# dselivanov/rsparse

Hardware: AMD Instinct MI355X
Metric: als_iterations_per_sec (higher is better)
Workload: dtype f32 (Gram products of rows > 512 / <= 32 non-zeros as 2 x fp16 / 3 x bf16 split terms of the fp32 operands, fp32 accumulate; everything else fp32)

## Files before the change

### rsparse_amd/csrc/wrmf_cgq.hip

```cpp
#include <algorithm>
#include <cstdlib>

#include "wrmf_internal.h"
#include "wrmf_device.h"

namespace rsparse_hip {
namespace {

using namespace dev;

typedef float f32x2 __attribute__((ext_vector_type(2)));

#ifndef RSP_ZPAD_MINCAPQ
#define RSP_ZPAD_MINCAPQ 0
#endif
#ifndef RSP_TSAVE_MINCAPQ
#define RSP_TSAVE_MINCAPQ 0
#endif
#ifndef RSP_GVFIRST_MINCAPQ
#define RSP_GVFIRST_MINCAPQ 16
#endif
#ifndef RSP_STREAM_IDX_PREFETCH
#define RSP_STREAM_IDX_PREFETCH 1
#endif
#ifndef RSP_IDX_PREFETCH_MAXWPR
#define RSP_IDX_PREFETCH_MAXWPR 2
#endif
#ifndef RSP_STREAM_PREFIX_Q
#define RSP_STREAM_PREFIX_Q 4
#endif

constexpr float kCgTolQ = 1e-10f;
constexpr int kMaxSavedSweeps = 4;

template <int KP>
struct QG {
  static constexpr int RPN = KP / 16;
  static constexpr int VW = RPN >= 4 ? 4 : RPN;
  static constexpr int NV = RPN / VW;
  __device__ static __forceinline__ int elem(int i, int r) { return (r / VW) * (16 * VW) + i * VW + (r % VW); }
};

template <int VW>
struct Piece;
template <>
struct Piece<4> { using type = float4; };
template <>
struct Piece<2> { using type = float2; };

__device__ __forceinline__ float row16_sum(float v) {
  v += dpp<0xB1>(v);
  v += dpp<0x4E>(v);
  v += dpp<0x141>(v);
  v += dpp<0x140>(v);
  return v;
}
__device__ __forceinline__ float groups_sum(float v) {
  {
    const unsigned u = __float_as_uint(v);
    const auto r = __builtin_amdgcn_permlane16_swap(u, u, false, false);
    v = __uint_as_float(r[0]) + __uint_as_float(r[1]);
  }
  {
    const unsigned u = __float_as_uint(v);
    const auto r = __builtin_amdgcn_permlane32_swap(u, u, false, false);
    v = __uint_as_float(r[0]) + __uint_as_float(r[1]);
  }
  return v;
}

__device__ __forceinline__ float groups_reduce_scatter4(const float a0, const float a1, const float a2, const float a3) {
  const auto s01 = __builtin_amdgcn_permlane16_swap(__float_as_uint(a0), __float_as_uint(a1), false, false);
  const float c = __uint_as_float(s01[0]) + __uint_as_float(s01[1]);
  const auto s23 = __builtin_amdgcn_permlane16_swap(__float_as_uint(a2), __float_as_uint(a3), false, false);
  const float d = __uint_as_float(s23[0]) + __uint_as_float(s23[1]);
  const auto t = __builtin_amdgcn_permlane32_swap(__float_as_uint(c), __float_as_uint(d), false, false);
  return __uint_as_float(t[0]) + __uint_as_float(t[1]);
}
__device__ __forceinline__ void groups_all_gather4(const float r, float& o0, float& o1, float& o2, float& o3) {
  const unsigned u = __float_as_uint(r);
  const auto h = __builtin_amdgcn_permlane32_swap(u, u, false, false);
  const auto lo = __builtin_amdgcn_permlane16_swap(h[0], h[0], false, false);
  const auto hi = __builtin_amdgcn_permlane16_swap(h[1], h[1], false, false);
  o0 = __uint_as_float(lo[0]);
  o1 = __uint_as_float(lo[1]);
  o2 = __uint_as_float(hi[0]);
  o3 = __uint_as_float(hi[1]);
}
#ifndef RSP_NO_GRS
#define RSP_GRS 1
#else
#define RSP_GRS 0
#endif

typedef _Float16 f16x2 __attribute__((ext_vector_type(2)));
typedef _Float16 f16x8 __attribute__((ext_vector_type(8)));
typedef float f32x4 __attribute__((ext_vector_type(4)));
__device__ __forceinline__ int fp16_scale_exp(float vmax) {
  const int eb = (int)((__float_as_uint(vmax) >> 23) & 0xffu);
  return min(253, max(1, 267 - eb));
}
__device__ __forceinline__ void split_f16(const float x0, const float x1, unsigned& hi, unsigned& lo) {
  const f32x2 v = {x0, x1};
  const f16x2 h = __builtin_convertvector(v, f16x2);
  const f32x2 r = v - __builtin_convertvector(h, f32x2);
  const f16x2 l = __builtin_convertvector(r, f16x2);
  hi = __builtin_bit_cast(unsigned, h);
  lo = __builtin_bit_cast(unsigned, l);
}
__device__ __forceinline__ float row16_max(float v) {
  v = fmaxf(v, dpp<0xB1>(v));
  v = fmaxf(v, dpp<0x4E>(v));
  v = fmaxf(v, dpp<0x141>(v));
  v = fmaxf(v, dpp<0x140>(v));
  return v;
}

__device__ __forceinline__ unsigned lds_addr(const void* p) {
  return (unsigned)(reinterpret_cast<uintptr_t>(p));
}
__device__ __forceinline__ void dma4(const void* g, unsigned lds_base) {
  asm volatile("s_mov_b32 m0, %1\n\ts_nop 0\n\tglobal_load_lds_dword %0, off" : : "v"(g), "s"(lds_base) : "memory", "m0");
}
__device__ __forceinline__ void wait_vm0() { asm volatile("s_waitcnt vmcnt(0)" ::: "memory"); }

template <int KP, int CAPQ, int WAVES, int WPR, int STREAM, bool IMPLICIT, int DMF = 0>
struct QSmem {
  static constexpr size_t gram_floats = (IMPLICIT && DMF != 1) ? (size_t)KP * KP : 0;
  static constexpr size_t vec_floats = IMPLICIT ? (size_t)WAVES * KP : 0;
  static constexpr size_t red_floats = WPR > 1 ? (size_t)2 * WAVES * KP + 2 * WAVES : 0;
  static constexpr size_t tsv_floats = (STREAM && !(RSP_STREAM_IDX_PREFETCH && IMPLICIT)) ? 0 : (size_t)WAVES * 2 * CAPQ * 4;
  static constexpr size_t pre_floats = STREAM ? (size_t)WAVES * RSP_STREAM_PREFIX_Q * 4 * KP : 0;
  static constexpr int dmf_ps = KP + 8, dmf_os = KP + 4;
  static constexpr size_t dmf_floats = DMF ? (size_t)WAVES * dmf_ps + (size_t)WAVES * dmf_os : 0;
  static constexpr size_t pfx_floats = (!STREAM && WPR > RSP_IDX_PREFETCH_MAXWPR && CAPQ * 4 == 64) ? (size_t)WAVES * 2 * 64 : 0;
  static constexpr size_t bytes = (gram_floats + vec_floats + red_floats + tsv_floats + pre_floats + dmf_floats + pfx_floats) * 4 + 16;
};

template <int KP, int CAPQ, int WAVES, int WPR, int STREAM, bool IMPLICIT, int DMF = 0, bool GB = false, bool KFULL = false>
__global__ __launch_bounds__(WAVES * 64, 2) void als_cgq_kernel(AlsArgs a, const int32_t* __restrict__ rows, int n_rows,
                                                             int rows_per_team, size_t loss_slot0) {
  using G_ = QG<KP>;
  constexpr int RPN = G_::RPN, VW = G_::VW, NV = G_::NV, CAP = CAPQ * 4, TEAMS = WAVES / WPR;
  using piece_t = typename Piece<VW>::type;
  using SM = QSmem<KP, CAPQ, WAVES, WPR, STREAM, IMPLICIT, DMF>;
  static_assert(WAVES % WPR == 0, "teams must tile the workgroup");
  constexpr bool GRS = RSP_GRS && RPN == 8 && VW == 4;
  auto groups_all_reduce8 = [](float(&a8)[RPN]) {
    if constexpr (RPN == 8) {
      const float r0 = groups_reduce_scatter4(a8[0], a8[1], a8[2], a8[3]);
      const float r1 = groups_reduce_scatter4(a8[4], a8[5], a8[6], a8[7]);
      groups_all_gather4(r0, a8[0], a8[1], a8[2], a8[3]);
      groups_all_gather4(r1, a8[4], a8[5], a8[6], a8[7]);
    }
  };
  static_assert(!DMF || (IMPLICIT && KP == 128 && WAVES == 4 && WPR == 1 && STREAM == 0), "DMF geometry");
  static_assert(DMF != 1 || CAPQ == 8, "register-resident G terms: only the 8-quad kernel has the 64 registers");
  static_assert(!GB || IMPLICIT, "the global bias of explicit feedback is removed from the data (R/model_WRMF.R:278-282)");
  const float gbias = GB ? a.gbias : 0.f, ltgt = GB ? a.loss_tgt_const : 1.f;
  extern __shared__ __attribute__((aligned(16))) char smem[];
  float* sG = reinterpret_cast<float*>(smem);
  float* sVec = sG + SM::gram_floats;
  float* sRed = sVec + SM::vec_floats;
  float* sRedL = sRed + (WPR > 1 ? 2 * WAVES * KP : 0);
  float* sTsv = sVec + SM::vec_floats + SM::red_floats;
  float* sPre = sTsv + SM::tsv_floats;
  float* sPfx = sPre + SM::pre_floats;
  _Float16* sPh = reinterpret_cast<_Float16*>(sPre + SM::pre_floats);
  _Float16* sPl = sPh + WAVES * SM::dmf_ps;
  float* sOut = reinterpret_cast<float*>(sPl + WAVES * SM::dmf_ps);

  const int tid = threadIdx.x, lane = tid & 63, wv = rfl(tid >> 6);
  const int g = lane >> 4, i = lane & 15;
  const int team = wv / WPR, tw = wv % WPR;
  const int k = KFULL ? KP : a.k;
  if constexpr (IMPLICIT && DMF == 0) {
    constexpr int GU = (KP * KP) % (8 * WAVES * 64) == 0 ? 8 : ((KP * KP) % (2 * WAVES * 64) == 0 ? 2 : 1);
    static_assert((KP * KP) % (GU * WAVES * 64) == 0, "the Gramian copy walks whole batches");
    for (int e0 = tid; e0 < KP * KP; e0 += GU * WAVES * 64) {
      float gv[GU];
#pragma unroll
      for (int u = 0; u < GU; u++) {
        const int e = e0 + u * WAVES * 64, r = e / KP, c = e % KP;
        gv[u] = a.XtX[(size_t)min(r, k - 1) * k + min(c, k - 1)];
      }
#pragma unroll
      for (int u = 0; u < GU; u++) {
        const int e = e0 + u * WAVES * 64, r = e / KP, c = e % KP;
        sG[e] = (r < k && c < k) ? gv[u] : 0.f;
      }
    }
  }
  for (int e = tid; e < (int)(SM::vec_floats + SM::red_floats + SM::tsv_floats); e += WAVES * 64) sVec[e] = 0.f;
  __syncthreads();

  constexpr int NRES = (IMPLICIT && CAPQ == 8 && WPR == 1 && !STREAM && KP == 128 && !DMF) ? 2 : 0;
  piece_t gres[NRES > 0 ? NRES : 1][4][NV];
  if constexpr (NRES > 0) {
#pragma unroll
    for (int rs = 0; rs < NRES; rs++)
#pragma unroll
      for (int u = 0; u < 4; u++)
#pragma unroll
        for (int b = 0; b < NV; b++)
          gres[rs][u][b] = *reinterpret_cast<const piece_t*>(sG + (4 * (g + 4 * rs) + u) * KP + b * 16 * VW + i * VW);
  }
  f16x8 gAh[DMF == 1 ? 2 : 1][DMF == 1 ? 4 : 1], gAl[DMF == 1 ? 2 : 1][DMF == 1 ? 4 : 1];
  char* sGf = reinterpret_cast<char*>(sG) + (size_t)wv * 16 * 1024;
  float ginv = 1.f;
  if constexpr (DMF) {
    const int m = lane & 15, kb = lane >> 4;
    float gmax = 0.f;
#pragma unroll
    for (int t = 0; t < 2; t++)
#pragma unroll
      for (int ks = 0; ks < 4; ks++)
#pragma unroll
        for (int e = 0; e < 8; e++) {
          const int r = 32 * wv + 16 * t + m, c = 32 * ks + 8 * kb + e;
          {
            const float gv = a.XtX[(size_t)min(r, k - 1) * k + min(c, k - 1)];
            gmax = fmaxf(gmax, fabsf(gv) * ((r < k && c < k) ? 1.f : 0.f));
          }
        }
    for (int o = 32; o > 0; o >>= 1) gmax = fmaxf(gmax, __shfl_xor(gmax, o));
    const int ge = fp16_scale_exp(gmax);
    const float gs = __uint_as_float((unsigned)ge << 23);
    ginv = __uint_as_float((unsigned)(254 - ge) << 23);
#pragma unroll
    for (int t = 0; t < 2; t++)
#pragma unroll
      for (int ks = 0; ks < 4; ks++) {
        unsigned hi[4], lo[4];
#pragma unroll
        for (int e = 0; e < 8; e += 2) {
          const int r = 32 * wv + 16 * t + m, c = 32 * ks + 8 * kb + e;
          const float g0v = a.XtX[(size_t)min(r, k - 1) * k + min(c, k - 1)];
          const float g0 = g0v * ((r < k && c < k) ? 1.f : 0.f);
          const float g1v = a.XtX[(size_t)min(r, k - 1) * k + min(c + 1, k - 1)];
          const float g1 = g1v * ((r < k && c + 1 < k) ? 1.f : 0.f);
          split_f16(g0 * gs, g1 * gs, hi[e / 2], lo[e / 2]);
        }
        const uint4 h4 = {hi[0], hi[1], hi[2], hi[3]}, l4 = {lo[0], lo[1], lo[2], lo[3]};
        if constexpr (DMF == 1) {
          gAh[t][ks] = __builtin_bit_cast(f16x8, h4);
          gAl[t][ks] = __builtin_bit_cast(f16x8, l4);
        } else {
          *reinterpret_cast<uint4*>(sGf + ((t * 4 + ks) * 2 + 0) * 1024 + lane * 16) = h4;
          *reinterpret_cast<uint4*>(sGf + ((t * 4 + ks) * 2 + 1) * 1024 + lane * 16) = l4;
        }
      }
    if constexpr (DMF == 2) wave_sync();
  }
  float* vec = sVec + wv * KP;
  float* tacc = sTsv + wv * 2 * CAP;
  float* tcur = tacc + CAP;
  int buf = 0;
  double wloss = 0.0;
#ifdef RSP_CGQ_PROF
  unsigned long long cq_t[6] = {0, 0, 0, 0, 0, 0};
  unsigned long long cq_l = __builtin_amdgcn_s_memtime();
#define CQ_T(j) { const unsigned long long t1_ = __builtin_amdgcn_s_memtime(); cq_t[j] += t1_ - cq_l; cq_l = t1_; }
#else
#define CQ_T(j)
#endif
  int pf_id = 0, pf_cnt = -1;
  float pf_c = 0.f;
  const int team_global = blockIdx.x * TEAMS + team;
  const int total_teams = gridDim.x * TEAMS;

  auto row_index = [&](int itn) { return team_global + itn * total_teams; };
  int row_c = 0, p1_c = 0, p2_c = 0, row_n = 0;
  if (rows_per_team > 0 && row_index(0) < n_rows) {
    row_c = rows[row_index(0)];
    p1_c = a.col_ptrs[row_c];
    p2_c = a.col_ptrs[row_c + 1];
  }
  if (rows_per_team > 1 && row_index(1) < n_rows) row_n = rows[row_index(1)];
  for (int it = 0; it < rows_per_team; ++it) {
    const int ri = row_index(it);
    const bool have = ri < n_rows;
    if (WPR == 1 && !DMF && !have) break;
    const int row = have ? rfl(row_c) : 0;
    const int p1 = have ? rfl(p1_c) : 0;
    const int p2 = have ? rfl(p2_c) : 0;
    {
      int p1_n = 0, p2_n = 0, row_nn = 0;
      if (it + 1 < rows_per_team && row_index(it + 1) < n_rows) {
        p1_n = a.col_ptrs[row_n];
        p2_n = a.col_ptrs[row_n + 1];
      }
      if (it + 2 < rows_per_team && row_index(it + 2) < n_rows) row_nn = rows[row_index(it + 2)];
      row_c = row_n;
      p1_c = p1_n;
      p2_c = p2_n;
      row_n = row_nn;
    }
    const int cnt = p2 - p1;
    float* yrow = a.Y + (size_t)row * k;
    if (!GB && WPR == 1 && cnt <= 0) {
      if (!DMF || have)
        for (int e = lane; e < k; e += 64) yrow[e] = 0.f;
      if constexpr (!DMF) continue;
    }
    constexpr int PQ = STREAM ? RSP_STREAM_PREFIX_Q : 0, PCAP = PQ * 4, PTEAM = PCAP * WPR;
    const int pre = STREAM ? min(cnt, PTEAM) : 0;
    const int pw = STREAM ? max(0, min(PCAP, pre - tw * PCAP)) : 0;
    const int nchunks = (cnt - pre + CAP - 1) / CAP;
    constexpr bool resident = STREAM == 0;
    const float lam_use =
        IMPLICIT ? 0.f : (float)(a.lambda_loss * (a.dynamic_lambda ? (double)(float)cnt : 1.0));

    float* tscr = nullptr;
    float alph[kMaxSavedSweeps];
#pragma unroll
    for (int s2 = 0; s2 < kMaxSavedSweeps; s2++) alph[s2] = 0.f;
    if constexpr (STREAM == 1) {
      if (a.tscr && have && a.cg_steps <= kMaxSavedSweeps) tscr = a.tscr + a.stream_off[ri];
    }

    float xt[CAPQ][RPN];
    float cv[CAPQ];
    constexpr int NSL = (CAP + 63) / 64;
    float cl[NSL];
#pragma unroll
    for (int s2 = 0; s2 < NSL; s2++) cl[s2] = 0.f;
    int ccnt = 0;

    constexpr bool ZPAD = STREAM == 0 && CAPQ >= RSP_ZPAD_MINCAPQ;
    constexpr bool TSAVE = STREAM == 0 && CAPQ >= RSP_TSAVE_MINCAPQ;
    constexpr bool GVFIRST = STREAM == 0 && CAPQ >= RSP_GVFIRST_MINCAPQ;
    constexpr bool IDXPF = CAP <= 64 && ((STREAM == 0 && WPR <= RSP_IDX_PREFETCH_MAXWPR) || (STREAM == 1 && IMPLICIT && RSP_STREAM_IDX_PREFETCH));
#ifdef RSP_NO_DMAPF
    constexpr bool DMAPF = false;
#else
    constexpr bool DMAPF = KFULL && !IDXPF && SM::pfx_floats > 0;
#endif
    int* pfxI = reinterpret_cast<int*>(sPfx) + wv * 128;
    float* pfxC = sPfx + wv * 128 + 64;
    int pf_pos = -1;
    auto gather_q = [&](auto nq_tag, const int base, const int n, const bool from_pf = false) {
      constexpr int NQG = decltype(nq_tag)::value;
      int id[NQG > 0 ? NQG : 1];
      if constexpr (DMAPF) {
        if (!from_pf && n > 0) {
          const int j = base + min(lane, n - 1);
          dma4(a.row_idx + j, lds_addr(pfxI));
          dma4(a.vals + j, lds_addr(pfxC));
          wait_vm0();
        }
        wave_sync();
#pragma unroll
        for (int q = 0; q < NQG; q++) {
          const int j = max(min(4 * q + g, n - 1), 0);
          id[q] = pfxI[j];
          cv[q] = (!ZPAD || 4 * q + g < n) ? pfxC[j] : 0.f;
        }
        if constexpr (TSAVE) cl[0] = lane < n ? pfxC[lane] : 0.f;
        wave_sync();
      } else if (IDXPF && from_pf) {
        int* xi = reinterpret_cast<int*>(tacc);
        wave_sync();
        xi[lane & (CAP - 1)] = pf_id;
        tcur[lane & (CAP - 1)] = pf_c;
        wave_sync();
#pragma unroll
        for (int q = 0; q < NQG; q++) {
          const int j = max(min(4 * q + g, n - 1), 0);
          id[q] = xi[j];
          cv[q] = (!ZPAD || 4 * q + g < n) ? tcur[j] : 0.f;
        }
        if constexpr (TSAVE) cl[0] = lane < n ? pf_c : 0.f;
        wave_sync();
      } else {
#pragma unroll
        for (int q = 0; q < NQG; q++) {
          const int j = max(min(4 * q + g, n - 1), 0);
          id[q] = a.row_idx[base + j];
          const float c = a.vals[base + j];
          cv[q] = (!ZPAD || 4 * q + g < n) ? c : 0.f;
        }
        if constexpr (TSAVE) {
#pragma unroll
          for (int s2 = 0; s2 < NSL; s2++) cl[s2] = lane + 64 * s2 < n ? a.vals[base + lane + 64 * s2] : 0.f;
        }
      }
#pragma unroll
      for (int q = 0; q < NQG; q++) {
        const float* src = (!ZPAD || 4 * q + g < n) ? a.X + (size_t)id[q] * k : a.zero_row;
#pragma unroll
        for (int b = 0; b < NV; b++) {
          const int off = b * 16 * VW + i * VW;
          if constexpr (KFULL) {
            const piece_t pc = *reinterpret_cast<const piece_t*>(src + off);
            const float* pf = reinterpret_cast<const float*>(&pc);
#pragma unroll
            for (int c = 0; c < VW; c++) xt[q][b * VW + c] = pf[c];
          } else {
            const piece_t pc = *reinterpret_cast<const piece_t*>(src + min(off, k - VW));
            const float* pf = reinterpret_cast<const float*>(&pc);
#pragma unroll
            for (int c = 0; c < VW; c++) xt[q][b * VW + c] = off < k ? pf[c] : 0.f;
          }
        }
      }
    };
    auto gather = [&](const int base, const int n, const bool from_pf = false) {
      gather_q(std::integral_constant<int, CAPQ>{}, base, n, from_pf);
    };
    float* pre_lds = sPre + (size_t)wv * PQ * 4 * KP + g * KP;
    auto prefix_chunk = [&](const bool first) {
      if constexpr (PQ > 0) {
        const int base = p1 + tw * PCAP;
        if (first) {
          gather_q(std::integral_constant<int, PQ>{}, base, pw);
#pragma unroll
          for (int q = 0; q < PQ; q++)
#pragma unroll
            for (int b = 0; b < NV; b++) {
              piece_t pc;
              float* pf = reinterpret_cast<float*>(&pc);
#pragma unroll
              for (int c = 0; c < VW; c++) pf[c] = xt[q][b * VW + c];
              *reinterpret_cast<piece_t*>(pre_lds + q * 4 * KP + b * 16 * VW + i * VW) = pc;
            }
        } else {
#pragma unroll
          for (int q = 0; q < PQ; q++) cv[q] = a.vals[base + min(4 * q + g, pw - 1)];
#pragma unroll
          for (int q = 0; q < PQ; q++)
#pragma unroll
            for (int b = 0; b < NV; b++) {
              const piece_t pc = *reinterpret_cast<const piece_t*>(pre_lds + q * 4 * KP + b * 16 * VW + i * VW);
              const float* pf = reinterpret_cast<const float*>(&pc);
#pragma unroll
              for (int c = 0; c < VW; c++) xt[q][b * VW + c] = pf[c];
            }
        }
      }
    };

    float x[RPN], r[RPN], p[RPN], ap[RPN];
    auto load_warm_start = [&]() {
#pragma unroll
      for (int b = 0; b < NV; b++) {
        const int off = b * 16 * VW + i * VW;
        piece_t pc;
        float* pf = reinterpret_cast<float*>(&pc);
#pragma unroll
        for (int c = 0; c < VW; c++) pf[c] = 0.f;
        if (have && off < k) pc = *reinterpret_cast<const piece_t*>(yrow + off);
#pragma unroll
        for (int c = 0; c < VW; c++) x[b * VW + c] = pf[c];
      }
    };
    constexpr bool WS_FIRST = KFULL && resident;
    if constexpr (WS_FIRST) load_warm_start();
    if constexpr (resident) {
#ifdef RSP_SEQ_FILL
      const int per = CAP;
#else
      const int per = min(CAP, (((cnt + WPR - 1) / WPR) + 15) & ~15);
#endif
      ccnt = max(0, min(per, cnt - tw * per));
#ifdef RSP_GATHER_PRIO
      __builtin_amdgcn_s_setprio(3);
#endif
      if constexpr (WS_FIRST) {
        gather(ccnt > 0 ? p1 + tw * per : p1, ccnt, ccnt > 0 && pf_cnt == ccnt);
      } else {
        if (ccnt > 0) gather(p1 + tw * per, ccnt, pf_cnt == ccnt);
      }
      pf_cnt = -1;
#ifdef RSP_GATHER_PRIO
      __builtin_amdgcn_s_setprio(0);
#endif
    }

    CQ_T(0)
    if constexpr (!WS_FIRST) load_warm_start();

    auto quad_pass = [&](const float(&v)[RPN], const int mode, float(&acc)[RPN], float& lacc, float* tsave) {
      float* trec = (mode == 0 ? tacc : tcur) + g;
      constexpr int QB = 4;
#pragma unroll
      for (int q0 = 0; q0 < CAPQ; q0 += QB) {
        if (4 * q0 < ccnt) {
          float t[QB];
#ifndef RSP_NO_QUAD_ILV
          f32x2 s2[QB];
#pragma unroll
          for (int u = 0; u < QB; u++) s2[u] = f32x2{0.f, 0.f};
#pragma unroll
          for (int rr = 0; rr < RPN; rr += 2) {
            const f32x2 va = {v[rr], v[rr + 1]};
#pragma unroll
            for (int u = 0; u < QB; u++) {
              const f32x2 xa = {xt[q0 + u][rr], xt[q0 + u][rr + 1]};
              s2[u] = __builtin_elementwise_fma(xa, va, s2[u]);
            }
          }
#pragma unroll
          for (int u = 0; u < QB; u++) t[u] = s2[u].x + s2[u].y;
#pragma unroll
          for (int u = 0; u < QB; u++) t[u] += dpp<0xB1>(t[u]);
#pragma unroll
          for (int u = 0; u < QB; u++) t[u] += dpp<0x4E>(t[u]);
#pragma unroll
          for (int u = 0; u < QB; u++) t[u] += dpp<0x141>(t[u]);
#pragma unroll
          for (int u = 0; u < QB; u++) t[u] += dpp<0x140>(t[u]);
#else
#pragma unroll
          for (int u = 0; u < QB; u++) {
            f32x2 s2 = {0.f, 0.f};
#pragma unroll
            for (int rr = 0; rr < RPN; rr += 2) {
              const f32x2 xa = {xt[q0 + u][rr], xt[q0 + u][rr + 1]};
              const f32x2 va = {v[rr], v[rr + 1]};
              s2 = __builtin_elementwise_fma(xa, va, s2);
            }
            t[u] = s2.x + s2.y;
          }
#pragma unroll
          for (int u = 0; u < QB; u++) t[u] = row16_sum(t[u]);
#endif
#pragma unroll
          for (int u = 0; u < QB; u++) {
            const int q = q0 + u;
            const bool valid = ZPAD || 4 * q + g < ccnt;
            const float c = cv[q];
            if constexpr (STREAM == 1) {
              if (tsave && valid && i == 0) tsave[4 * q + g] = t[u];
            } else if constexpr (TSAVE) {
              trec[4 * q] = t[u];
            }
            if (mode == 2) {
              const float d = IMPLICIT ? ltgt - t[u] : c - t[u];
              lacc += valid ? (IMPLICIT ? c * d * d : d * d) : 0.f;
            } else {
              float w;
              if (mode == 0) w = IMPLICIT ? c - (c - 1.f) * (GB ? t[u] + gbias : t[u]) : c - t[u];
              else w = IMPLICIT ? (c - 1.f) * t[u] : t[u];
              w = valid ? w : 0.f;
#pragma unroll
              for (int rr = 0; rr < RPN; rr++) acc[rr] = fmaf(w, xt[q][rr], acc[rr]);
            }
          }
        }
      }
    };

    auto sweep = [&](const float(&v)[RPN], const int mode, float(&out)[RPN], float& loss_out, const bool live,
                     const int sidx = 0) {
      float acc[RPN];
#pragma unroll
      for (int rr = 0; rr < RPN; rr++) acc[rr] = 0.f;
      float lacc = 0.f;
      float vinv = 0.f;
      if constexpr (DMF) {
        if (mode != 2) {
          float vmax = 0.f;
#pragma unroll
          for (int rr = 0; rr < RPN; rr++) vmax = fmaxf(vmax, fabsf(v[rr]));
          vmax = row16_max(vmax);
          const int ve = fp16_scale_exp(vmax);
          const float vs = __uint_as_float((unsigned)ve << 23);
          vinv = __uint_as_float((unsigned)(254 - ve) << 23) * (mode == 0 ? -1.f : 1.f);
          if (g < NV) {
            float w4[VW];
#pragma unroll
            for (int c = 0; c < VW; c++) w4[c] = (g == 0 ? v[c] : v[VW + c]) * vs;
            unsigned h0, l0, h1, l1;
            split_f16(w4[0], w4[1], h0, l0);
            split_f16(w4[2], w4[3], h1, l1);
            const int off = wv * SM::dmf_ps + g * 16 * VW + i * VW;
            *reinterpret_cast<uint2*>(sPh + off) = make_uint2(h0, h1);
            *reinterpret_cast<uint2*>(sPl + off) = make_uint2(l0, l1);
          }
          __syncthreads();
          f32x4 d0[2], d1[2];
#pragma unroll
          for (int t = 0; t < 2; t++) d0[t] = d1[t] = f32x4{0.f, 0.f, 0.f, 0.f};
          const int nb = (lane & 3) * SM::dmf_ps + 8 * (lane >> 4);
#pragma unroll
          for (int ks = 0; ks < 4; ks++) {
            const f16x8 bh = *reinterpret_cast<const f16x8*>(sPh + nb + 32 * ks);
            const f16x8 bl = *reinterpret_cast<const f16x8*>(sPl + nb + 32 * ks);
#pragma unroll
            for (int t = 0; t < 2; t++) {
              f16x8 ah, al;
              if constexpr (DMF == 1) {
                ah = gAh[t][ks];
                al = gAl[t][ks];
              } else {
                ah = *reinterpret_cast<const f16x8*>(sGf + ((t * 4 + ks) * 2 + 0) * 1024 + lane * 16);
                al = *reinterpret_cast<const f16x8*>(sGf + ((t * 4 + ks) * 2 + 1) * 1024 + lane * 16);
              }
              d0[t] = __builtin_amdgcn_mfma_f32_16x16x32_f16(ah, bh, d0[t], 0, 0, 0);
              d1[t] = __builtin_amdgcn_mfma_f32_16x16x32_f16(ah, bl, d1[t], 0, 0, 0);
              d1[t] = __builtin_amdgcn_mfma_f32_16x16x32_f16(al, bh, d1[t], 0, 0, 0);
            }
          }
          if ((lane & 15) < 4) {
#pragma unroll
            for (int t = 0; t < 2; t++) {
              const f32x4 d = (d0[t] + d1[t]) * ginv;
              *reinterpret_cast<f32x4*>(sOut + (lane & 15) * SM::dmf_os + 32 * wv + 16 * t + 4 * (lane >> 4)) = d;
            }
          }
        }
      }
      if (live) {
        if constexpr (IMPLICIT && !DMF) {
          if (mode != 2) {
            wave_sync();
            if (g == 0) {
#pragma unroll
              for (int b = 0; b < NV; b++) {
                piece_t pc;
                float* pf = reinterpret_cast<float*>(&pc);
#pragma unroll
                for (int c = 0; c < VW; c++) pf[c] = v[b * VW + c];
                *reinterpret_cast<piece_t*>(vec + b * 16 * VW + i * VW) = pc;
              }
            }
            wave_sync();
          }
        }
        auto dense_part = [&]() {
          if (IMPLICIT && !DMF && mode != 2) {
            const float sign = mode == 0 ? -1.f : 1.f;
            if constexpr (NRES > 0) {
#pragma unroll
              for (int rs = 0; rs < NRES; rs++) {
                const int kk = 4 * (g + 4 * rs);
                const float4 vb = *reinterpret_cast<const float4*>(vec + kk);
                const float vv[4] = {sign * vb.x, sign * vb.y, sign * vb.z, sign * vb.w};
#pragma unroll
                for (int u = 0; u < 4; u++)
#pragma unroll
                  for (int b = 0; b < NV; b++) {
                    const float* pf = reinterpret_cast<const float*>(&gres[rs][u][b]);
#pragma unroll
                    for (int c = 0; c < VW; c++) acc[b * VW + c] = fmaf(vv[u], pf[c], acc[b * VW + c]);
                  }
              }
            }
            for (int s4 = tw * 4 + g + 4 * NRES; s4 < KP / 4; s4 += WPR * 4) {
              const int kk = 4 * s4;
              const float4 vb = *reinterpret_cast<const float4*>(vec + kk);
              const float vv[4] = {sign * vb.x, sign * vb.y, sign * vb.z, sign * vb.w};
#pragma unroll
              for (int u = 0; u < 4; u++) {
                const float* grow = sG + (kk + u) * KP;
#pragma unroll
                for (int b = 0; b < NV; b++) {
                  const piece_t pc = *reinterpret_cast<const piece_t*>(grow + b * 16 * VW + i * VW);
                  const float* pf = reinterpret_cast<const float*>(&pc);
#pragma unroll
                  for (int c = 0; c < VW; c++) acc[b * VW + c] = fmaf(vv[u], pf[c], acc[b * VW + c]);
                }
              }
            }
          }
        };
        if constexpr (GVFIRST) dense_part();
        if (resident) {
          if (mode != 2 || !TSAVE) {
            quad_pass(v, mode, acc, lacc, nullptr);
          } else {
            wave_sync();
            float esum = 0.f;
#pragma unroll
            for (int s2 = 0; s2 < NSL; s2++) {
              const int sl = NSL == 1 ? (lane & (CAP - 1)) : lane + 64 * s2;
              const float t = tacc[sl];
              const float clv = cl[s2];
              const float d = IMPLICIT ? ltgt - t : clv - t;
              const float e = IMPLICIT ? clv * d * d : d * d;
              esum += lane + 64 * s2 < ccnt ? e : 0.f;
            }
            lacc = row16_sum(esum);
          }
        } else if (mode == 2 && tscr) {
          for (int ch = tw; ch < (cnt + CAP - 1) / CAP; ch += WPR) {
            const int n = min(CAP, cnt - ch * CAP);
            if (lane < n) {
              const size_t pos = (size_t)ch * CAP + lane;
              float t = tscr[pos];
#pragma unroll
              for (int s2 = 0; s2 < kMaxSavedSweeps; s2++)
                if (s2 < a.cg_steps) t = fmaf(alph[s2], tscr[(size_t)(s2 + 1) * a.stream_nnz + pos], t);
              const float c = a.vals[p1 + pos];
              const float d = IMPLICIT ? ltgt - t : c - t;
              lacc += IMPLICIT ? c * d * d : d * d;
            }
          }
          lacc = row16_sum(lacc);
        } else {
          if (pw > 0) {
            prefix_chunk(mode == 0);
            ccnt = pw;
            quad_pass(v, mode, acc, lacc, tscr ? tscr + (size_t)sidx * a.stream_nnz + (size_t)tw * PCAP : nullptr);
          }
          for (int ch = tw; ch < nchunks; ch += WPR) {
            ccnt = min(CAP, cnt - pre - ch * CAP);
            gather(p1 + pre + ch * CAP, ccnt, IDXPF && pf_pos == ch && pf_cnt == ccnt);
            if constexpr (IDXPF) {
              const int nch = ch + WPR < nchunks ? ch + WPR : tw;
              const int ncc = min(CAP, cnt - pre - nch * CAP);
              const int j = p1 + pre + nch * CAP + min(lane & (CAP - 1), ncc - 1);
              pf_id = a.row_idx[j];
              pf_c = a.vals[j];
              pf_cnt = ncc;
              pf_pos = nch;
            }
            quad_pass(v, mode, acc, lacc,
                      tscr ? tscr + (size_t)sidx * a.stream_nnz + (size_t)pre + (size_t)ch * CAP : nullptr);
          }
        }
        if constexpr (!GVFIRST) dense_part();
        if constexpr (!DMF) {
          if (mode != 2) {
            if constexpr (GRS) {
              if constexpr (WPR == 1) groups_all_reduce8(acc);
            } else {
#pragma unroll
              for (int rr = 0; rr < RPN; rr++) acc[rr] = groups_sum(acc[rr]);
            }
          } else {
            lacc = groups_sum(lacc);
          }
        }
      }
      if constexpr (DMF) {
        if (mode != 2) {
          __syncthreads();
          const float f = g == 0 ? vinv : 0.f;
#pragma unroll
          for (int b = 0; b < NV; b++) {
            const f32x4 o = *reinterpret_cast<const f32x4*>(sOut + wv * SM::dmf_os + b * 16 * VW + i * VW);
#pragma unroll
            for (int c = 0; c < VW; c++) acc[b * VW + c] = fmaf(f, o[c], acc[b * VW + c]);
          }
          if constexpr (GRS) {
            groups_all_reduce8(acc);
          } else {
#pragma unroll
            for (int rr = 0; rr < RPN; rr++) acc[rr] = groups_sum(acc[rr]);
          }
        } else {
          lacc = groups_sum(lacc);
        }
      }
      if constexpr (WPR > 1) {
        float* red = sRed + buf * WAVES * KP;
        if (mode != 2) {
          if constexpr (GRS) {
            const float r0 = groups_reduce_scatter4(acc[0], acc[1], acc[2], acc[3]);
            const float r1 = groups_reduce_scatter4(acc[4], acc[5], acc[6], acc[7]);
            red[wv * KP + 4 * i + g] = r0;
            red[wv * KP + 64 + 4 * i + g] = r1;
          } else if (g == 0) {
#pragma unroll
            for (int b = 0; b < NV; b++) {
              piece_t pc;
              float* pf = reinterpret_cast<float*>(&pc);
#pragma unroll
              for (int c = 0; c < VW; c++) pf[c] = acc[b * VW + c];
              *reinterpret_cast<piece_t*>(red + wv * KP + b * 16 * VW + i * VW) = pc;
            }
          }
        } else if (lane == 0) {
          sRedL[buf * WAVES + wv] = lacc;
        }
        __syncthreads();
        if (mode != 2) {
#pragma unroll
          for (int rr = 0; rr < RPN; rr++) acc[rr] = 0.f;
#pragma unroll
          for (int w2 = 0; w2 < WPR; w2++) {
#pragma unroll
            for (int b = 0; b < NV; b++) {
              const piece_t pc = *reinterpret_cast<const piece_t*>(red + (team * WPR + w2) * KP + b * 16 * VW + i * VW);
              const float* pf = reinterpret_cast<const float*>(&pc);
#pragma unroll
              for (int c = 0; c < VW; c++) acc[b * VW + c] += pf[c];
            }
          }
        } else {
          lacc = 0.f;
#pragma unroll
          for (int w2 = 0; w2 < WPR; w2++) lacc += sRedL[buf * WAVES + team * WPR + w2];
        }
        buf ^= 1;
      } else {
        __builtin_amdgcn_sched_barrier(0);
      }
      if (mode != 2) {
#pragma unroll
        for (int rr = 0; rr < RPN; rr++) out[rr] = acc[rr];
        if constexpr (GB) {
          if (mode == 0) {
#pragma unroll
            for (int b = 0; b < NV; b++) {
              const int off = b * 16 * VW + i * VW;
              const piece_t pc = *reinterpret_cast<const piece_t*>(a.rhs_init + min(off, k - VW));
              const float* pf = reinterpret_cast<const float*>(&pc);
#pragma unroll
              for (int c = 0; c < VW; c++) out[b * VW + c] += off < k ? pf[c] : 0.f;
            }
          }
        }
        if constexpr (!IMPLICIT) {
#pragma unroll
          for (int rr = 0; rr < RPN; rr++) out[rr] = fmaf(mode == 0 ? -lam_use : lam_use, v[rr], out[rr]);
        }
      } else {
        loss_out = lacc;
      }
    };

    auto dot16 = [&](const float(&u)[RPN], const float(&w)[RPN]) {
// ... 8 lines not shown
    CQ_T(1)
    sweep(x, 0, r, dummy, live);
    CQ_T(2)
    if constexpr (IDXPF && STREAM == 0) {
      if (it + 1 < rows_per_team && row_index(it + 1) < n_rows) {
        const int np1 = rfl(p1_c), ncnt = rfl(p2_c) - np1;
        const int nper = min(CAP, (((ncnt + WPR - 1) / WPR) + 15) & ~15);
        const int ncc = max(0, min(nper, ncnt - tw * nper));
        if (ncc > 0) {
          const int j = np1 + tw * nper + min(lane & (CAP - 1), ncc - 1);
          pf_id = a.row_idx[j];
          pf_c = a.vals[j];
          pf_cnt = ncc;
        }
      }
    }
    if constexpr (DMAPF) {
      if (it + 1 < rows_per_team && row_index(it + 1) < n_rows) {
        const int np1 = rfl(p1_c), ncnt = rfl(p2_c) - np1;
        const int nper = min(CAP, (((ncnt + WPR - 1) / WPR) + 15) & ~15);
        const int ncc = max(0, min(nper, ncnt - tw * nper));
        if (ncc > 0) {
          const int j = np1 + tw * nper + min(lane, ncc - 1);
          dma4(a.row_idx + j, lds_addr(pfxI));
          dma4(a.vals + j, lds_addr(pfxC));
          pf_cnt = ncc;
        }
      }
    }
    CQ_T(3)
#pragma unroll
    for (int rr = 0; rr < RPN; rr++) p[rr] = r[rr];
    float rsold = dot16(r, r);
    bool conv = false;
    for (int itc = 0; itc < a.cg_steps; ++itc) {
      if (WPR == 1 && !DMF && conv) break;
      CQ_T(4)
      sweep(p, 1, ap, dummy, live && !conv, itc + 1);
      CQ_T(2)
      CQ_T(3)
      if (!conv) {
        const float pap = dot16(p, ap);
        const float alpha = (float)((double)rsold / (double)pap);
#pragma unroll
        for (int s2 = 0; s2 < kMaxSavedSweeps; s2++)
          if (s2 == itc) alph[s2] = alpha;
        if constexpr (TSAVE) {
          wave_sync();
#pragma unroll
          for (int s2 = 0; s2 < NSL; s2++) {
            const int sl = NSL == 1 ? (lane & (CAP - 1)) : lane + 64 * s2;
            tacc[sl] = fmaf(alpha, tcur[sl], tacc[sl]);
          }
          wave_sync();
        }
#pragma unroll
        for (int rr = 0; rr < RPN; rr++) {
          x[rr] = fmaf(alpha, p[rr], x[rr]);
          r[rr] = fmaf(-alpha, ap[rr], r[rr]);
        }
        const float rsnew = dot16(r, r);
        if (rsnew < kCgTolQ) {
          conv = true;
        } else {
          const float beta = (float)((double)rsnew / (double)rsold);
#pragma unroll
          for (int rr = 0; rr < RPN; rr++) p[rr] = fmaf(p[rr], beta, r[rr]);
          rsold = rsnew;
        }
      }
    }
    float rl = 0.f;
    CQ_T(4)
    sweep(x, 2, ap, rl, live);
    CQ_T(2)
    if constexpr (DMAPF) wait_vm0();
    if constexpr (IDXPF && STREAM == 0) {
      asm volatile("" : "+v"(pf_id), "+v"(pf_c));
    }
    if (live && tw == 0) {
      const float xx = dot16(x, x);
      wloss += IMPLICIT ? (double)rl + a.lambda_loss * (double)xx : (double)(rl + lam_use * xx);
      if (g == 0) {
#pragma unroll
        for (int b = 0; b < NV; b++) {
          const int off = b * 16 * VW + i * VW;
          if (off < k) {
            piece_t pc;
            float* pf = reinterpret_cast<float*>(&pc);
#pragma unroll
            for (int c = 0; c < VW; c++) pf[c] = x[b * VW + c];
            *reinterpret_cast<piece_t*>(yrow + off) = pc;
          }
        }
      }
    }
  }
  CQ_T(5)
#ifdef RSP_CGQ_PROF
  if (WAVES == 8 && WPR == 8 && !STREAM && a.ne_prof && lane == 0)
    for (int j = 0; j < 6; j++) atomicAdd(a.ne_prof + (size_t)65536 * 80 - 16 + j, cq_t[j]);
#endif
  if (lane == 0) a.loss_partials[loss_slot0 + (size_t)blockIdx.x * WAVES + wv] = wloss;
}

struct BucketDef { int waves, wpr, capq, stream, max_len; };
constexpr int kNB = 6;
constexpr int kNCfg = 2;
constexpr BucketDef kBuckets[kNCfg][kNB] = {
    {{8, 8, 16, 1, 0x7fffffff}, {8, 8, 16, 0, 512}, {4, 4, 16, 0, 256}, {4, 2, 16, 0, 128}, {4, 1, 16, 0, 64}, {4, 1, 8, 0, 32}},
    {{8, 8, 16, 1, 0x7fffffff}, {4, 4, 32, 0, 512}, {4, 2, 32, 0, 256}, {4, 1, 32, 0, 128}, {4, 1, 16, 0, 64}, {4, 1, 8, 0, 32}},
};
constexpr int cfg_of_kp(int KP) { return KP == 64 ? 1 : 0; }

bool dense_mfma_enabled() {
#ifdef RSP_AB
  static const bool on = [] {
    const char* e = std::getenv("RSPARSE_HIP_DENSE_MFMA");
    return !(e && e[0] == '0');
  }();
  return on;
#else
  return true;
#endif
}

bool kfull_enabled() {
#ifdef RSP_AB
  static const bool on = [] {
    const char* e = std::getenv("RSPARSE_HIP_KFULL");
    return !(e && e[0] == '0');
  }();
  return on;
#else
  return true;
#endif
}

template <int KP, int WAVES, int CAPQ, int WPR, int STREAM, bool IMPLICIT, bool GB, int DMF = 0, bool KFULL = false>
hipError_t launch_bucket(const AlsArgs& a, const int32_t* rows, int n_rows, int grid, size_t slot0, hipStream_t s,
                         hipEvent_t* ev_slot) {
  if (n_rows <= 0) return hipSuccess;
  constexpr bool kDmfGeometry = IMPLICIT && KP == 128 && WAVES == 4 && WPR == 1 && (CAPQ == 8 || CAPQ == 16) && STREAM == 0;
  if constexpr (kDmfGeometry && !DMF) {
    if (dense_mfma_enabled())
      return launch_bucket<KP, WAVES, CAPQ, WPR, STREAM, IMPLICIT, GB, CAPQ == 8 ? 1 : 2>(a, rows, n_rows, grid, slot0, s, ev_slot);
  }
  if constexpr (!KFULL && STREAM == 0) {
    if (a.k == KP && kfull_enabled())
      return launch_bucket<KP, WAVES, CAPQ, WPR, STREAM, IMPLICIT, GB, DMF, true>(a, rows, n_rows, grid, slot0, s, ev_slot);
  }
  constexpr int TEAMS = WAVES / WPR;
  auto kern = als_cgq_kernel<KP, CAPQ, WAVES, WPR, STREAM, IMPLICIT, DMF, GB, KFULL>;
  const size_t lds = QSmem<KP, CAPQ, WAVES, WPR, STREAM, IMPLICIT, DMF>::bytes;
  hipError_t err = hipFuncSetAttribute(reinterpret_cast<const void*>(kern),
                                       hipFuncAttributeMaxDynamicSharedMemorySize, (int)lds);
  if (err != hipSuccess) return err;
  const int total_teams = grid * TEAMS;
  const int rpt = (n_rows + total_teams - 1) / total_teams;
  prof_note(ev_slot, reinterpret_cast<const void*>(kern));
  hipLaunchKernelGGL(kern, dim3(grid), dim3(WAVES * 64), lds, s, a, rows, n_rows, rpt, slot0);
  return hipGetLastError();
}

struct BucketStreams {
  hipStream_t st[kNB] = {nullptr, nullptr, nullptr, nullptr, nullptr, nullptr};
  hipEvent_t fork = nullptr, fork0 = nullptr;
  hipEvent_t done[kNB] = {nullptr, nullptr, nullptr, nullptr, nullptr, nullptr};
  int device = -1;
  hipError_t ensure() {
    int dev = 0;
    hipError_t err = hipGetDevice(&dev);
    if (err != hipSuccess) return err;
    if (dev == device) return hipSuccess;
    device = dev;
    if ((err = hipEventCreateWithFlags(&fork, hipEventDisableTiming)) != hipSuccess) return err;
    if ((err = hipEventCreateWithFlags(&fork0, hipEventDisableTiming)) != hipSuccess) return err;
    for (int b = 0; b < kNB; b++) {
      if ((err = hipStreamCreateWithFlags(&st[b], hipStreamNonBlocking)) != hipSuccess) return err;
      if ((err = hipEventCreateWithFlags(&done[b], hipEventDisableTiming)) != hipSuccess) return err;
    }
    return hipSuccess;
  }
};
thread_local BucketStreams g_bs;

int g_launch_mode = 2;
int concurrent_buckets() { return g_launch_mode; }

size_t bucket_slots(const QSchedule& q, int b, int k, bool implicit) {
  const int cfg = cfg_of_kp(padded_rank(k));
  const BucketDef d = kBuckets[cfg][b];
  if (d.wpr <= 0) return 0;
  if (d.stream && ne_supported(k)) return (size_t)(q.ne_entries + q.ne_nsplit) + (size_t)(q.mf_n > 0 ? cg_mf_loss_slots(q.mf_n) : 0);
  const int rows = q.off[b + 1] - q.off[b];
  if (b == kNB - 1 && rows > 0 && cgp_supported(k, implicit) && dense_mfma_enabled()) {
    const int split = std::min(std::max(q.pair_first, q.off[b]), q.off[b + 1]);
    return (size_t)cgq_bucket_grid(split - q.off[b], b, cfg) * d.waves + (size_t)cgp_grid(q.off[b + 1] - split) * 4;
  }
  return (size_t)cgq_bucket_grid(rows, b, cfg) * d.waves;
}

template <int KP, int CFG, bool IMPLICIT, bool GB>
hipError_t launch_all(const AlsArgs& a, const QSchedule& q, hipStream_t s, hipEvent_t* ev) {
  hipError_t err;
  size_t slot = 0;
  const int cmode = ev ? 0 : concurrent_buckets();
  const bool overlap = cmode != 0;
  bool forked = false;
  if (overlap) {
    if ((err = g_bs.ensure()) != hipSuccess) return err;
  }
#define RSP_BUCKET(B)                                                                                       \
  {                                                                                                         \
    constexpr BucketDef D = kBuckets[CFG][B];                                                               \
    if (ev && (err = hipEventRecord(ev[B], s)) != hipSuccess) return err;                                   \
    if constexpr (D.wpr > 0) {                                                                              \
      const int n = q.off[B + 1] - q.off[B];                                                                \
      const int grid = cgq_bucket_grid(n, B, CFG);                                                          \
      if (n > 0) {                                                                                          \
        hipStream_t bs = s;                                                                                 \
        const bool side = overlap && !(cmode == 2 && D.stream);                                             \
        if (side) {                                                                                         \
          if (!forked) {                                                                                    \
            if ((err = hipEventRecord(g_bs.fork, s)) != hipSuccess) return err;                             \
            forked = true;                                                                                  \
          }                                                                                                 \
          bs = g_bs.st[B];                                                                                  \
          if ((err = hipStreamWaitEvent(bs, g_bs.fork, 0)) != hipSuccess) return err;                       \
        }                                                                                                   \
        if (D.stream && ne_supported(a.k)) {                                                                \
           \
           \
           \
           \
          const bool mside = overlap && q.ne_wg > 0 && q.mf_n > 0;                                          \
           \
          if (mside && (err = hipEventRecord(g_bs.fork0, s)) != hipSuccess) return err;                     \
          if (q.ne_wg > 0 &&                                                                                \
              (err = launch_als_ne(a, q, IMPLICIT, a.loss_partials + slot, bs, q.mf_n > 0 ? nullptr : (ev ? ev + B : nullptr))) != hipSuccess) \
            return err;                                                                                     \
          if (q.mf_n > 0) {                                                                                 \
            hipStream_t ms = bs;                                                                            \
            if (mside) {                                                                                    \
              ms = g_bs.st[B];                                                                              \
              if ((err = hipStreamWaitEvent(ms, g_bs.fork0, 0)) != hipSuccess) return err;                  \
            }                                                                                               \
            if ((err = launch_als_cg_mf(a, q.mf_rows, q.mf_n, (int)(slot + (size_t)(q.ne_entries + q.ne_nsplit)), ms, \
                                        ev ? ev + B : nullptr)) != hipSuccess)                              \
              return err;                                                                                   \
            if (mside) {                                                                                    \
              if ((err = hipEventRecord(g_bs.done[B], ms)) != hipSuccess) return err;                       \
              if ((err = hipStreamWaitEvent(s, g_bs.done[B], 0)) != hipSuccess) return err;                 \
            }                                                                                               \
          }                                                                                                 \
        } else if constexpr (D.stream && KP > 32) {        \
          return hipErrorInvalidValue;                                                                      \
        } else if (B == kNB - 1 && cgp_supported(a.k, IMPLICIT) && dense_mfma_enabled()) {                    \
           \
          const int first = q.off[B], split = std::min(std::max(q.pair_first, first), q.off[B + 1]);         \
          const int n_main = split - first, n_pair = q.off[B + 1] - split;                                   \
          const int g_main = cgq_bucket_grid(n_main, B, CFG);                                                \
          if ((err = launch_bucket<KP, D.waves, D.capq, D.wpr, D.stream, IMPLICIT, GB>(a, q.order + first, n_main, g_main, slot, \
                                                                                  bs, ev ? ev + B : nullptr)) != hipSuccess) \
            return err;                                                                                     \
          if ((err = launch_als_cgp(a, q.order + split, n_pair, slot + (size_t)g_main * D.waves, bs,          \
                                    n_main > 0 ? nullptr : (ev ? ev + B : nullptr))) != hipSuccess)           \
            return err;                                                                                     \
        } else if ((err = launch_bucket<KP, D.waves, D.capq, D.wpr, D.stream, IMPLICIT, GB>(a, q.order + q.off[B], n, grid, slot, \
                                                                                bs, ev ? ev + B : nullptr)) != hipSuccess) \
          return err;                                                                                       \
        if (side) {                                                                                         \
          if ((err = hipEventRecord(g_bs.done[B], bs)) != hipSuccess) return err;                           \
          if ((err = hipStreamWaitEvent(s, g_bs.done[B], 0)) != hipSuccess) return err;                     \
        }                                                                                                   \
      }                                                                                                     \
      slot += bucket_slots(q, B, a.k, IMPLICIT);                                                             \
    }                                                                                                       \
  }
  RSP_BUCKET(0)
  RSP_BUCKET(1)
  RSP_BUCKET(2)
  RSP_BUCKET(3)
  RSP_BUCKET(4)
  RSP_BUCKET(5)
#undef RSP_BUCKET
  if (ev && (err = hipEventRecord(ev[kNB], s)) != hipSuccess) return err;
  return hipSuccess;
}

}

int cgq_num_buckets() { return kNB; }
int cgq_bucket_wpr(int cfg, int b) { return kBuckets[cfg][b].wpr; }
int cgq_bucket_capq(int cfg, int b) { return kBuckets[cfg][b].capq; }
int cgq_bucket_waves(int cfg, int b) { return kBuckets[cfg][b].waves; }
int cgq_bucket_stream(int cfg, int b) { return kBuckets[cfg][b].stream; }

int cgq_bucket_grid(int n_rows, int b, int cfg) {
  const BucketDef d = kBuckets[cfg][b];
  if (n_rows <= 0 || d.wpr <= 0) return 0;
  const int teams = d.waves / d.wpr;
  const int base = d.stream ? 16 : (d.wpr == 1 ? 64 : (d.wpr == 2 ? 64 : 32));
  int rows_per_team = base;
  const long spread = (long)teams * 512;
  if ((long)n_rows < spread * rows_per_team) rows_per_team = (int)((n_rows + spread - 1) / spread);
  if (rows_per_team < 1) rows_per_team = 1;
// ... 39 lines not shown
```

Before: 8.004.

## Partition implicit-feedback row entries by confidence to skip zero-weight CG dot products

In the implicit, full-k, resident CG kernel, each row's non-zeros are split with wave ballots into entries whose confidence differs from 1 and entries equal to 1. Those are compacted into LDS staging with the active ones first. For confidence-1 entries the (c-1) weight vanishes, so the mode-1 quad pass runs only over active entries and mode 0 applies a plain c*x accumulation to the passive ones. The loss pass recomputes dot products for passive entries only. An optional deal mode (off by default) redistributes active and passive entries across the waves of a team. The cost is extra ballot, compaction and LDS traffic per row gather, and the saving depends on how many confidences are exactly 1.

Result: faster. 8.113, median of 6 (+1.4%).

```diff
diff --git a/rsparse_amd/csrc/wrmf_cgq.hip b/rsparse_amd/csrc/wrmf_cgq.hip
--- a/rsparse_amd/csrc/wrmf_cgq.hip
+++ b/rsparse_amd/csrc/wrmf_cgq.hip
@@ -124,7 +124,14 @@
 }
 __device__ __forceinline__ void wait_vm0() { asm volatile("s_waitcnt vmcnt(0)" ::: "memory"); }
 
-template <int KP, int CAPQ, int WAVES, int WPR, int STREAM, bool IMPLICIT, int DMF = 0>
+#ifndef RSP_PART_MAXWPR
+#define RSP_PART_MAXWPR 2
+#endif
+constexpr bool part_on(bool implicit, bool kfull, bool gb, int stream, int wpr) {
+  return implicit && kfull && !gb && stream == 0 && wpr <= RSP_PART_MAXWPR;
+}
+
+template <int KP, int CAPQ, int WAVES, int WPR, int STREAM, bool IMPLICIT, int DMF = 0, bool PART = false>
 struct QSmem {
   static constexpr size_t gram_floats = (IMPLICIT && DMF != 1) ? (size_t)KP * KP : 0;
   static constexpr size_t vec_floats = IMPLICIT ? (size_t)WAVES * KP : 0;
@@ -134,7 +141,13 @@
   static constexpr int dmf_ps = KP + 8, dmf_os = KP + 4;
   static constexpr size_t dmf_floats = DMF ? (size_t)WAVES * dmf_ps + (size_t)WAVES * dmf_os : 0;
   static constexpr size_t pfx_floats = (!STREAM && WPR > RSP_IDX_PREFETCH_MAXWPR && CAPQ * 4 == 64) ? (size_t)WAVES * 2 * 64 : 0;
-  static constexpr size_t bytes = (gram_floats + vec_floats + red_floats + tsv_floats + pre_floats + dmf_floats + pfx_floats) * 4 + 16;
+#ifdef RSP_PART_DEAL
+  static constexpr size_t stg_floats = (PART && WPR > 1) ? (size_t)WAVES * 2 * CAPQ * 4 + WAVES : 0;
+#else
+  static constexpr size_t stg_floats = 0;
+#endif
+  static constexpr size_t bytes =
+      (gram_floats + vec_floats + red_floats + tsv_floats + pre_floats + dmf_floats + pfx_floats + stg_floats) * 4 + 16;
 };
 
 template <int KP, int CAPQ, int WAVES, int WPR, int STREAM, bool IMPLICIT, int DMF = 0, bool GB = false, bool KFULL = false>
@@ -143,7 +156,13 @@
   using G_ = QG<KP>;
   constexpr int RPN = G_::RPN, VW = G_::VW, NV = G_::NV, CAP = CAPQ * 4, TEAMS = WAVES / WPR;
   using piece_t = typename Piece<VW>::type;
-  using SM = QSmem<KP, CAPQ, WAVES, WPR, STREAM, IMPLICIT, DMF>;
+  constexpr bool PART = part_on(IMPLICIT, KFULL, GB, STREAM, WPR);
+#ifdef RSP_PART_DEAL
+  constexpr bool DEAL = PART && WPR > 1;
+#else
+  constexpr bool DEAL = false;
+#endif
+  using SM = QSmem<KP, CAPQ, WAVES, WPR, STREAM, IMPLICIT, DMF, PART>;
   static_assert(WAVES % WPR == 0, "teams must tile the workgroup");
   constexpr bool GRS = RSP_GRS && RPN == 8 && VW == 4;
   auto groups_all_reduce8 = [](float(&a8)[RPN]) {
@@ -169,6 +188,7 @@
   _Float16* sPh = reinterpret_cast<_Float16*>(sPre + SM::pre_floats);
   _Float16* sPl = sPh + WAVES * SM::dmf_ps;
   float* sOut = reinterpret_cast<float*>(sPl + WAVES * SM::dmf_ps);
+  float* sStg = reinterpret_cast<float*>(smem) + (SM::bytes - 16) / 4 - SM::stg_floats;
 
   const int tid = threadIdx.x, lane = tid & 63, wv = rfl(tid >> 6);
   const int g = lane >> 4, i = lane & 15;
@@ -326,6 +346,8 @@
 #pragma unroll
     for (int s2 = 0; s2 < NSL; s2++) cl[s2] = 0.f;
     int ccnt = 0;
+    int nact = 0;
+    int share = CAP;
 
     constexpr bool ZPAD = STREAM == 0 && CAPQ >= RSP_ZPAD_MINCAPQ;
     constexpr bool TSAVE = STREAM == 0 && CAPQ >= RSP_TSAVE_MINCAPQ;
@@ -342,7 +364,127 @@
     auto gather_q = [&](auto nq_tag, const int base, const int n, const bool from_pf = false) {
       constexpr int NQG = decltype(nq_tag)::value;
       int id[NQG > 0 ? NQG : 1];
-      if constexpr (DMAPF) {
+      int nv = n;
+      if constexpr (PART) {
+        static_assert(NQG == CAPQ, "PART: resident rows only");
+        int li[NSL];
+        float lc[NSL];
+        if constexpr (DMAPF) {
+          static_assert(NSL == 1, "DMAPF: 64 slots");
+          if (!from_pf && n > 0) {
+            dma4(a.row_idx + base + min(lane, n - 1), lds_addr(pfxI));
+            dma4(a.vals + base + min(lane, n - 1), lds_addr(pfxC));
+            wait_vm0();
+          }
+          wave_sync();
+          li[0] = pfxI[max(min(lane, n - 1), 0)];
+          lc[0] = lane < n ? pfxC[lane] : 0.f;
+        } else if (IDXPF && from_pf) {
+          static_assert(!IDXPF || NSL == 1, "IDXPF: <= 64 slots");
+          li[0] = pf_id;
+          lc[0] = lane < n ? pf_c : 0.f;
+        } else {
+#pragma unroll
+          for (int s2 = 0; s2 < NSL; s2++) {
+            const int j = base + max(min(lane + 64 * s2, n - 1), 0);
+            li[s2] = a.row_idx[j];
+            const float c = a.vals[j];
+            lc[s2] = lane + 64 * s2 < n ? c : 0.f;
+          }
+        }
+        unsigned long long ma[NSL], mp[NSL];
+        int na = 0;
+#pragma unroll
+        for (int s2 = 0; s2 < NSL; s2++) {
+          const bool in = lane + 64 * s2 < n;
+          ma[s2] = __builtin_amdgcn_ballot_w64(in && lc[s2] != 1.f);
+          mp[s2] = __builtin_amdgcn_ballot_w64(in && lc[s2] == 1.f);
+          na += __builtin_popcountll(ma[s2]);
+        }
+        int* stI = !DEAL ? reinterpret_cast<int*>(tacc) : reinterpret_cast<int*>(sStg) + wv * 2 * CAP;
+        float* stC = !DEAL ? tcur : sStg + wv * 2 * CAP + CAP;
+        wave_sync();
+        {
+          int ra = 0, rp = na;
+#pragma unroll
+          for (int s2 = 0; s2 < NSL; s2++) {
+            const unsigned lo_a = (unsigned)ma[s2], hi_a = (unsigned)(ma[s2] >> 32);
+            const unsigned lo_p = (unsigned)mp[s2], hi_p = (unsigned)(mp[s2] >> 32);
+            const int ia = ra + (int)__builtin_amdgcn_mbcnt_hi(hi_a, __builtin_amdgcn_mbcnt_lo(lo_a, 0u));
+            const int ip = rp + (int)__builtin_amdgcn_mbcnt_hi(hi_p, __builtin_amdgcn_mbcnt_lo(lo_p, 0u));
+            if (lane + 64 * s2 < n) {
+              const int pos = lc[s2] != 1.f ? ia : ip;
+              stI[pos] = li[s2];
+              stC[pos] = lc[s2];
+            }
+            ra += __builtin_popcountll(ma[s2]);
+            rp += __builtin_popcountll(mp[s2]);
+          }
+        }
+        if constexpr (!DEAL) {
+          nact = rfl(na);
+          wave_sync();
+#pragma unroll
+          for (int s2 = 0; s2 < NSL; s2++) cl[s2] = lane + 64 * s2 < n ? stC[lane + 64 * s2] : 0.f;
+        } else {
+          if (lane == 0) reinterpret_cast<int*>(sStg)[WAVES * 2 * CAP + wv] = na;
+          __syncthreads();
+          const int* tn = reinterpret_cast<const int*>(sStg) + WAVES * 2 * CAP + team * WPR;
+          const float* tb = sStg + team * WPR * 2 * CAP;
+          int nau[WPR];
+          int A = 0;
+#pragma unroll
+          for (int u = 0; u < WPR; u++) {
+            nau[u] = rfl(tn[u]);
+            A += nau[u];
+          }
+          const int P = cnt - A, T = (cnt + WPR - 1) / WPR, pa = (A + WPR - 1) / WPR;
+          const int a_w = max(0, min(pa, A - tw * pa));
+          const int po = tw * T - min(A, tw * pa);
+          const int p_w = max(0, min(T - a_w, P - po));
+          nv = a_w + p_w;
+          nact = a_w;
+          ccnt = nv;
+          int li2[NSL];
+          float lc2[NSL];
+#pragma unroll
+          for (int s2 = 0; s2 < NSL; s2++) {
+            const int s = lane + 64 * s2, ga = tw * pa + s, gp = po + s - a_w;
+            int srcA = 0, srcP = 0, accA = 0, accP = 0;
+#pragma unroll
+            for (int u = 0; u < WPR; u++) {
+              const int npu = max(0, min(share, cnt - u * share)) - nau[u];
+              if (ga >= accA && ga < accA + nau[u]) srcA = u * 2 * CAP + ga - accA;
+              if (gp >= accP && gp < accP + npu) srcP = u * 2 * CAP + nau[u] + gp - accP;
+              accA += nau[u];
+              accP += npu;
+            }
+            const int src = s < a_w ? srcA : srcP;
+            const int iv = reinterpret_cast<const int*>(tb)[src];
+            const float cv2 = tb[src + CAP];
+            li2[s2] = iv;
+            lc2[s2] = s < nv ? cv2 : 0.f;
+          }
+          static_assert(CAP % 64 == 0, "team shares are whole multiples of 64 slots");
+          stI = reinterpret_cast<int*>(tacc);
+          stC = tcur;
+          wave_sync();
+#pragma unroll
+          for (int s2 = 0; s2 < NSL; s2++) {
+            stI[lane + 64 * s2] = li2[s2];
+            stC[lane + 64 * s2] = lc2[s2];
+            cl[s2] = lc2[s2];
+          }
+          wave_sync();
+        }
+#pragma unroll
+        for (int q = 0; q < NQG; q++) {
+          const int j = max(min(4 * q + g, nv - 1), 0);
+          id[q] = stI[j];
+          cv[q] = 4 * q + g < nv ? stC[j] : 0.f;
+        }
+        wave_sync();
+      } else if constexpr (DMAPF) {
         if (!from_pf && n > 0) {
           const int j = base + min(lane, n - 1);
           dma4(a.row_idx + j, lds_addr(pfxI));
@@ -387,7 +529,7 @@
       }
 #pragma unroll
       for (int q = 0; q < NQG; q++) {
-        const float* src = (!ZPAD || 4 * q + g < n) ? a.X + (size_t)id[q] * k : a.zero_row;
+        const float* src = (!ZPAD || 4 * q + g < nv) ? a.X + (size_t)id[q] * k : a.zero_row;
 #pragma unroll
         for (int b = 0; b < NV; b++) {
           const int off = b * 16 * VW + i * VW;
@@ -463,6 +605,7 @@
       const int per = min(CAP, (((cnt + WPR - 1) / WPR) + 15) & ~15);
 #endif
       ccnt = max(0, min(per, cnt - tw * per));
+      share = per;
 #ifdef RSP_GATHER_PRIO
       __builtin_amdgcn_s_setprio(3);
 #endif
@@ -480,51 +623,63 @@
     CQ_T(0)
     if constexpr (!WS_FIRST) load_warm_start();
 
+    constexpr int QB = 4;
+    auto block_dots = [&](const float(&v)[RPN], const int q0, float(&t)[QB]) {
+#ifndef RSP_NO_QUAD_ILV
+      f32x2 s2[QB];
+#pragma unroll
+      for (int u = 0; u < QB; u++) s2[u] = f32x2{0.f, 0.f};
+#pragma unroll
+      for (int rr = 0; rr < RPN; rr += 2) {
+        const f32x2 va = {v[rr], v[rr + 1]};
+#pragma unroll
+        for (int u = 0; u < QB; u++) {
+          const f32x2 xa = {xt[q0 + u][rr], xt[q0 + u][rr + 1]};
+          s2[u] = __builtin_elementwise_fma(xa, va, s2[u]);
+        }
+      }
+#pragma unroll
+      for (int u = 0; u < QB; u++) t[u] = s2[u].x + s2[u].y;
+#pragma unroll
+      for (int u = 0; u < QB; u++) t[u] += dpp<0xB1>(t[u]);
+#pragma unroll
+      for (int u = 0; u < QB; u++) t[u] += dpp<0x4E>(t[u]);
+#pragma unroll
+      for (int u = 0; u < QB; u++) t[u] += dpp<0x141>(t[u]);
+#pragma unroll
+      for (int u = 0; u < QB; u++) t[u] += dpp<0x140>(t[u]);
+#else
+#pragma unroll
+      for (int u = 0; u < QB; u++) {
+        f32x2 s2 = {0.f, 0.f};
+#pragma unroll
+        for (int rr = 0; rr < RPN; rr += 2) {
+          const f32x2 xa = {xt[q0 + u][rr], xt[q0 + u][rr + 1]};
+          const f32x2 va = {v[rr], v[rr + 1]};
+          s2 = __builtin_elementwise_fma(xa, va, s2);
+        }
+        t[u] = s2.x + s2.y;
+      }
+#pragma unroll
+      for (int u = 0; u < QB; u++) t[u] = row16_sum(t[u]);
+#endif
+    };
+
     auto quad_pass = [&](const float(&v)[RPN], const int mode, float(&acc)[RPN], float& lacc, float* tsave) {
       float* trec = (mode == 0 ? tacc : tcur) + g;
-      constexpr int QB = 4;
+      const int qlim = (PART && mode == 1) ? nact : ccnt;
 #pragma unroll
       for (int q0 = 0; q0 < CAPQ; q0 += QB) {
-        if (4 * q0 < ccnt) {
+        if (PART && mode == 0 && 4 * q0 >= nact && 4 * q0 < ccnt) {
+#pragma unroll
+          for (int u = 0; u < QB; u++) {
+            const float c = cv[q0 + u];
+#pragma unroll
+            for (int rr = 0; rr < RPN; rr++) acc[rr] = fmaf(c, xt[q0 + u][rr], acc[rr]);
+          }
+        } else if (4 * q0 < qlim) {
           float t[QB];
-#ifndef RSP_NO_QUAD_ILV
-          f32x2 s2[QB];
-#pragma unroll
-          for (int u = 0; u < QB; u++) s2[u] = f32x2{0.f, 0.f};
-#pragma unroll
-          for (int rr = 0; rr < RPN; rr += 2) {
-            const f32x2 va = {v[rr], v[rr + 1]};
-#pragma unroll
-            for (int u = 0; u < QB; u++) {
-              const f32x2 xa = {xt[q0 + u][rr], xt[q0 + u][rr + 1]};
-              s2[u] = __builtin_elementwise_fma(xa, va, s2[u]);
-            }
-          }
-#pragma unroll
-          for (int u = 0; u < QB; u++) t[u] = s2[u].x + s2[u].y;
-#pragma unroll
-          for (int u = 0; u < QB; u++) t[u] += dpp<0xB1>(t[u]);
-#pragma unroll
-          for (int u = 0; u < QB; u++) t[u] += dpp<0x4E>(t[u]);
-#pragma unroll
-          for (int u = 0; u < QB; u++) t[u] += dpp<0x141>(t[u]);
-#pragma unroll
-          for (int u = 0; u < QB; u++) t[u] += dpp<0x140>(t[u]);
-#else
-#pragma unroll
-          for (int u = 0; u < QB; u++) {
-            f32x2 s2 = {0.f, 0.f};
-#pragma unroll
-            for (int rr = 0; rr < RPN; rr += 2) {
-              const f32x2 xa = {xt[q0 + u][rr], xt[q0 + u][rr + 1]};
-              const f32x2 va = {v[rr], v[rr + 1]};
-              s2 = __builtin_elementwise_fma(xa, va, s2);
-            }
-            t[u] = s2.x + s2.y;
-          }
-#pragma unroll
-          for (int u = 0; u < QB; u++) t[u] = row16_sum(t[u]);
-#endif
+          block_dots(v, q0, t);
 #pragma unroll
           for (int u = 0; u < QB; u++) {
             const int q = q0 + u;
@@ -670,6 +825,18 @@
           if (mode != 2 || !TSAVE) {
             quad_pass(v, mode, acc, lacc, nullptr);
           } else {
+            if constexpr (PART) {
+#pragma unroll
+              for (int q0 = 0; q0 < CAPQ; q0 += QB) {
+                if (4 * q0 < ccnt && 4 * q0 + 4 * QB > nact) {
+                  float t[QB];
+                  block_dots(v, q0, t);
+#pragma unroll
+                  for (int u = 0; u < QB; u++)
+                    if (4 * (q0 + u) + g >= nact) tacc[4 * (q0 + u) + g] = t[u];
+                }
+              }
+            }
             wave_sync();
             float esum = 0.f;
 #pragma unroll
@@ -984,7 +1151,7 @@
   }
   constexpr int TEAMS = WAVES / WPR;
   auto kern = als_cgq_kernel<KP, CAPQ, WAVES, WPR, STREAM, IMPLICIT, DMF, GB, KFULL>;
-  const size_t lds = QSmem<KP, CAPQ, WAVES, WPR, STREAM, IMPLICIT, DMF>::bytes;
+  const size_t lds = QSmem<KP, CAPQ, WAVES, WPR, STREAM, IMPLICIT, DMF, part_on(IMPLICIT, KFULL, GB, STREAM, WPR)>::bytes;
   hipError_t err = hipFuncSetAttribute(reinterpret_cast<const void*>(kern),
                                        hipFuncAttributeMaxDynamicSharedMemorySize, (int)lds);
   if (err != hipSuccess) return err;
```
